# BurntSushi/rust-snappy

Hardware: AMD Instinct MI355X
Metric: GiB/s uncompressed (compress + decompress) on zflat/uflat corpus (higher is better)
Workload: dtype u8

## Files before the change

rust-snappy_amd/csrc/snapmi_api.hip:

```cpp
#include <hip/hip_runtime.h>

#include <cstdarg>
#include <cstdio>
#include <cstdlib>
#include <cstring>
#include <new>
#include <string>
#include <vector>

#include "snapmi.h"
#include "snapmi_test.h"
#include "snapmi_ctx.hpp"
#include "snapmi_launch.hpp"
#include "snapmi_device.hpp"
#include "snapmi_kernels.hpp"

using namespace snapmi;

namespace {

void set_err(snapmi_error *e, int kind, uint64_t a = 0, uint64_t b = 0,
             uint64_t c = 0)
{
    if (e) {
// ... 270 lines not shown
        ctx->small_table_kernel = (int)value;
    else if (strcmp(name, "small_table_min_blocks") == 0 && value >= 1)
        ctx->small_table_min_blocks = (uint64_t)value;
    else if (strcmp(name, "small_batch_kernel") == 0 && value >= 0 &&
             value <= 2)
        ctx->small_batch_kernel = (int)value;
    else if (strcmp(name, "lane_speculate") == 0 && value >= 0 && value <= 1)
        ctx->lane_speculate = (int)value;
    else if (strcmp(name, "lane_tail_probes") == 0 && value >= 0 &&
             value <= 4)
        ctx->lane_tail_probes = (uint32_t)value;
    else if (strcmp(name, "lane_tail_idle_pct") == 0 && value >= 0 &&
             value <= 100)
        ctx->lane_tail_idle_pct = (uint32_t)value;
    else if (strcmp(name, "span_kernel") == 0 && value >= kSpanMin &&
             value <= 1)
        ctx->span_kernel = (int)value;
    else if (strcmp(name, "match_kernel") == 0 && value >= 0 && value <= 2)
        ctx->match_kernel = (int)value;
    else if (strcmp(name, "match_spans_ratio_pct") == 0 && value >= 1 &&
             value <= 200)
        ctx->match_spans_ratio_pct = (uint32_t)value;
    else if (strcmp(name, "release_scratch") == 0 && value >= 0 && value <= 1)
        ctx->release_scratch = (int)value;
    else if (strcmp(name, "batch_long_streams") == 0 && value >= 0 &&
             value <= 1)
        ctx->batch_long_streams = (int)value;
    else if (strcmp(name, "both_wave_cus") == 0 && value >= 0 &&
             value <= 4096)
        ctx->both_wave_cus = (uint32_t)value;
    else if (strcmp(name, "tiny_stream_kernel") == 0 && value >= 0 &&
             value <= 1)
        ctx->tiny_stream_kernel = (int)value;
    else if (strcmp(name, "small_stream_kernel") == 0 && value >= 0 &&
             value <= 2)
        ctx->small_stream_kernel = (int)value;
    else if (strcmp(name, "frame_parallel_walk_min") == 0 && value >= 0)
        ctx->frame_parallel_walk_min = (uint64_t)value;
    else if (strcmp(name, "host_copy_kernel") == 0 && value >= 0 && value <= 3)
        ctx->host_copy_kernel = (int)value;
    else if (strcmp(name, "host_encode_slice") == 0 && value >= (1 << 16))
        ctx->host_encode_slice = (uint64_t)value;
    else if (strcmp(name, "host_decode_slice_chunks") == 0 && value >= 1)
        ctx->host_decode_slice_chunks = (uint64_t)value;
    else if (strcmp(name, "host_batch_slice") == 0 && value >= (1 << 16))
        ctx->host_batch_slice = (uint64_t)value;
    else if (strcmp(name, "range_scratch_bytes") == 0 && value >= (128 << 10))
        ctx->range_scratch_bytes = (uint64_t)value;
    else if (strcmp(name, "write_scratch_bytes") == 0 &&
             value >= (int64_t)(kSlotBytes + kMaxBlock))
        ctx->write_scratch_bytes = (uint64_t)value;
    else if (strcmp(name, "decode_kernel") == 0 &&
             (value == 0 || (value == 2 && kDec2) || value == 3))
        ctx->decode_kernel = ctx->lds_store_order_ok ? (int)value : 0;
    else
        return fail_ctx(ctx, SNAPMI_E_ARGUMENT, "unknown option %s", name);
    return SNAPMI_OK;
}

#ifdef SNAPMI_TESTING
int snapmi_ctx_set_test_option(snapmi_ctx *ctx, const char *name,
                               int64_t value)
{
    if (!ctx || !name)
        return SNAPMI_E_ARGUMENT;
    if (strcmp(name, "lane_waves_per_cu") == 0 && value >= 1 && value <= 32)
        ctx->lane_waves_per_cu = (uint32_t)value;
    else if (strcmp(name, "decode_many_min") == 0 && value >= 0)
        ctx->decode_many_min = (uint64_t)value;
    else if (strcmp(name, "lane_speculate_max_blocks") == 0 && value >= 0)
        ctx->lane_speculate_max_blocks = (uint64_t)value;
    else if (strcmp(name, "lane_max_waves") == 0 && value >= 0 &&
             value <= 0x7FFFFFFF)
        ctx->lane_max_waves = (uint32_t)value;
    else if (strcmp(name, "frame_crc_side_stream") == 0 && value >= 0 &&
             value <= 1)
        ctx->frame_crc_side_stream = value != 0;
    else if (strcmp(name, "lane_tables_uncached") == 0 && value >= 0 &&
             value <= 1)
        ctx->lane_tables_uncached = (int)value;
    else if (strcmp(name, "lane_overlap_encode") == 0 && value >= 0 &&
             value <= 2)
        ctx->lane_overlap_encode = (int)value;
    else if (strcmp(name, "frame_walk_segment") == 0 && value >= (128 << 10))
        ctx->frame_walk_segment = (uint64_t)value;
    else if (strcmp(name, "lane_table_stride_kib") == 0 &&
             (value == 0 || (value >= 256 && value <= 4096 && value % 4 == 0)))
        ctx->lane_table_stride_kib = (uint32_t)value;
    else if (strcmp(name, "lane_table_probe") == 0 && value >= 0 &&
             value <= 1)
        ctx->lane_table_probe = value != 0;
    else if (strcmp(name, "lane_tables_renew") == 0 && value == 1) {
        if (ctx->lane_tables.p) {
            HIP_TRY(ctx, hipStreamSynchronize(ctx->stream));
            snapmi::free_lane_tables(ctx);
        }
    } else if (strcmp(name, "lane_epoch_preset") == 0 && value >= -1 &&
             value <= 0xFFFF)
        ctx->lane_epoch_preset = value;
    else if (strcmp(name, "index_build_route") == 0 && value >= 0 &&
             value <= 2)
        ctx->index_build_route = (uint32_t)value;
    else if (strcmp(name, "index_build_group_streams") == 0 && value >= 1 &&
             value <= 4096)
        ctx->index_build_group_streams = (uint32_t)value;
    else if (strcmp(name, "stream_seg_log2") == 0 &&
             (value == 0 || value == 10 || value == 12))
        ctx->stream_seg_log2 = (uint32_t)value;
    else if (strcmp(name, "stream_scan_segs") == 0 &&
             (value == 0 || value == 8 || value == 16 || value == 32 ||
              value == 64))
        ctx->stream_scan_segs = (uint32_t)value;
    else if (strcmp(name, "lds_order_ok") == 0 && value >= 0 && value <= 1)
        ctx->lds_order_ok = ctx->lds_order_hw && value != 0;
    else if (strcmp(name, "host_batch_direct_min") == 0 && value >= 0)
        ctx->host_batch_direct_min = (uint64_t)value;
    else if (strcmp(name, "host_batch_pack_to_host") == 0 && value >= 0 &&
             value <= 1)
        ctx->host_batch_pack_to_host = (int)value;
    else if (strcmp(name, "host_batch_listed") == 0 && value >= 0 &&
             value <= 1)
        ctx->host_batch_listed = (int)value;
    else
        return fail_ctx(ctx, SNAPMI_E_ARGUMENT, "unknown test option %s",
                        name);
    return SNAPMI_OK;
}
#endif

void *snapmi_host_alloc(size_t bytes)
{
    void *p = nullptr;
    if (hipHostMalloc(&p, bytes ? bytes : 1, hipHostMallocDefault) != hipSuccess) {
        (void)hipGetLastError();
        return nullptr;
    }
    return p;
}

void snapmi_host_free(void *p)
{
    if (p)
        (void)hipHostFree(p);
}

const char *snapmi_table_probe_log(const snapmi_ctx *ctx)
{
    return ctx ? ctx->probe_log.c_str() : "";
}

size_t snapmi_error_string(const snapmi_error *e, char *buf, size_t cap)
{
    char tmp[256];
    const unsigned long long a = e ? e->a : 0, b = e ? e->b : 0,
                             c = e ? e->c : 0;
    int n = 0;
    switch (e ? e->kind : -1) {
    case SNAPMI_TOO_BIG:
        n = snprintf(tmp, sizeof tmp,
                     "snappy: input buffer (size = %llu) is larger than "
                     "allowed (size = %llu)", a, b);
        break;
    case SNAPMI_BUFFER_TOO_SMALL:
        n = snprintf(tmp, sizeof tmp,
                     "snappy: output buffer (size = %llu) is smaller than "
                     "required (size = %llu)", a, b);
// ... 481 lines not shown
```

rust-snappy_amd/csrc/snapmi_compress.hip:

```cpp
#include <type_traits>

#include "snapmi_device.hpp"
#include "snapmi_kernels.hpp"
#include "snapmi_scan.hpp"
#include "snapmi_span.hpp"

namespace snapmi {

namespace {

__device__ __forceinline__ uint32_t hash32(uint32_t x, uint32_t shift)
{
    return (x * 0x1E35A7BDu) >> shift;
}

struct DeltaTable {
    uint32_t d[448];
};
constexpr DeltaTable make_delta()
{
    DeltaTable t{};
    uint32_t skip = 32, p = 0;
    for (int i = 0; i < 448; i++) {
        t.d[i] = p < 0x100000u ? p : 0x100000u;
// ... 161 lines not shown
        o += lt;
        gcptr in = src + P;
        const uint32_t Lp = (L + 15u) & ~15u;
        if (L && L <= 64 && P + Lp <= n) {
            u32x4 v0 = {0, 0, 0, 0}, v1 = v0, v2 = v0, v3 = v0;
            v0 = ld128g(in);
            if (L > 16)
                v1 = ld128g(in + 16);
            if (L > 32)
                v2 = ld128g(in + 32);
            if (L > 48)
                v3 = ld128g(in + 48);
            typedef __attribute__((address_space(1))) u32x4 g_u32x4;
            typedef g_u32x4 __attribute__((aligned(1))) g_u32x4u;
            if (L >= 16)
                *(g_u32x4u *)o = v0;
            if (L >= 32)
                *(g_u32x4u *)(o + 16) = v1;
            if (L >= 48)
                *(g_u32x4u *)(o + 32) = v2;
            if (L >= 64)
                *(g_u32x4u *)(o + 48) = v3;
            const uint32_t pk = L >> 4;
            const u32x4 pv = pk == 0 ? v0 : (pk == 1 ? v1 : (pk == 2 ? v2 : v3));
            gptr po = o + (L & ~15u);
            const uint32_t r = L & 15u;
            if (r >= 4)
                st32u(po, pv.x);
            if (r >= 8)
                st32u(po + 4, pv.y);
            if (r >= 12)
                st32u(po + 8, pv.z);
            const uint32_t tl = r & 3u, tb = r & ~3u;
            const uint32_t ti = r >> 2;
            const uint32_t tw =
                ti == 0 ? pv.x : (ti == 1 ? pv.y : (ti == 2 ? pv.z : pv.w));
            if (tl >= 1)
                po[tb] = (uint8_t)tw;
            if (tl >= 2)
                po[tb + 1] = (uint8_t)(tw >> 8);
            if (tl >= 3)
                po[tb + 2] = (uint8_t)(tw >> 16);
        } else if (L && L <= 64) {
            uint32_t i = 0;
            for (; i + 4 <= L; i += 4)
                st32u(o + i, ld32u(in + i));
            for (; i < L; i++)
                o[i] = in[i];
        }
        gptr oc = o + L;
        const uint8_t olo = (uint8_t)O, ohi = (uint8_t)(O >> 8);
        for (uint32_t i = 0; i < n64; i++) {
            oc[0] = (uint8_t)((63u << 2) | 2u);
            oc[1] = olo;
            oc[2] = ohi;
            oc += 3;
        }
        if (mid) {
            oc[0] = (uint8_t)((59u << 2) | 2u);
            oc[1] = olo;
            oc[2] = ohi;
            oc += 3;
        }
        if (fin == 2) {
            oc[0] = (uint8_t)(((O >> 8) << 5) | ((fin_len - 4) << 2) | 1u);
            oc[1] = olo;
        } else if (fin == 3) {
            oc[0] = (uint8_t)(((fin_len - 1) << 2) | 2u);
            oc[1] = olo;
            oc[2] = ohi;
        }
        uint64_t longs = __ballot(L > 64);
        while (longs) {
            const uint32_t j = (uint32_t)__builtin_ctzll(longs);
            longs &= longs - 1;
            const uint32_t Lj = rdlane(L, j);
            const uint32_t Pj = rdlane(P, j);
            const uint64_t oj = ((uint64_t)rdlane((uint32_t)((uintptr_t)o >> 32), j) << 32) |
                                rdlane((uint32_t)(uintptr_t)o, j);
            wave_copy<true>((gptr)(uintptr_t)oj, src + Pj, Lj, lane);
        }
    }
};

template <class P>
__device__ __forceinline__ uint32_t extend_match(P src, uint32_t n,
                                                 uint32_t c, uint32_t p,
                                                 uint32_t lane)
{
    uint32_t len = 0;
    const uint32_t room = n - p;
    for (uint32_t pos = 0;; pos += 4 * kWave) {
        const uint32_t off = pos + 4 * lane;
        uint32_t eq = 0;
        if (off < room) {
            const uint32_t pa = c + off, pb = p + off;
            const uint32_t ca = pa < n - 4 ? pa : n - 4;
            const uint32_t cb = pb < n - 4 ? pb : n - 4;
            const uint32_t va = ld32u(src + ca) >> (8 * (pa - ca));
            const uint32_t vb = ld32u(src + cb) >> (8 * (pb - cb));
            const uint32_t x = va ^ vb;
            eq = x ? ((uint32_t)__builtin_ctz(x) >> 3) : 4u;
            const uint32_t lim = room - off;
            eq = eq < lim ? eq : lim;
        }
        const uint64_t stop = __ballot(eq < 4);
        if (stop == 0) {
            len += 4 * kWave;
            continue;
        }
        const uint32_t f = (uint32_t)__builtin_ctzll(stop);
        return len + 4 * f + rdlane(eq, f);
    }
}


}

template <bool kLds>
__device__ __forceinline__ void compress_one_block(
    const CompressArgs &a, const uint32_t b, const uint32_t lane,
    const lptr16 table, const uint32_t tbase, const uint32_t c2,
    const uint32_t c3, const uint32_t cB, const uint32_t cBn,
    __attribute__((address_space(3))) uint8_t *lblock = nullptr)
{

    uint32_t lo = 0, hi = a.n_streams;
    if (b < a.n_streams && a.blk_first[b] == b && a.blk_first[b + 1] > b) {
        lo = b;
        hi = b + 1;
    }
    while (hi - lo > 1) {
        const uint32_t mid = (lo + hi) >> 1;
        if (a.blk_first[mid] <= b)
            lo = mid;
        else
            hi = mid;
    }
    const uint32_t st = lo;
    const uint32_t k = b - a.blk_first[st];
    const uint64_t total = a.in_lens[st];
    const uint64_t boff = (uint64_t)k * kMaxBlock;
    gcptr src = (gcptr)a.in_ptrs[st] + boff;
    const uint64_t avail = total - boff;
    const uint32_t n = avail < kMaxBlock ? (uint32_t)avail : kMaxBlock;

    gptr dst;
    if (k == 0) {
        dst = (gptr)a.out_ptrs[st];
        if (lane == 0) {
            uint64_t v = total;
            uint32_t i = 0;
            while (v >= 0x80) {
                dst[i++] = (uint8_t)v | 0x80;
                v >>= 7;
            }
            dst[i] = (uint8_t)v;
        }
        dst += varint_len(total);
    } else {
        const uint32_t slot = a.slot_first[st] + k - 1;
        if (slot >= a.host_slots)
            return;
        dst = (gptr)a.scratch + (uint64_t)slot * kSlotBytes;
    }
    TokenSink out;
// ... 2025 lines not shown
    a.lane_epochs[g] = epoch;
    PROF_TAIL(
    if (a.prof && lane == 0)
        atomicMax(&a.prof[kProfTail + 1], (unsigned long long)wall_clock64());
    )
#ifdef SNAPMI_TESTING
    if (kTail && lane == 0 && multi_rounds)
        atomicAdd(&a.tok_ctl[kTokCtlMultiRounds], multi_rounds);
#endif
}
}

#define SNAPMI_LANE_KERNEL(name, spec, tail)                                  \
    __global__ __launch_bounds__(64) void name(CompressArgs a)                \
    {                                                                         \
        __shared__ __attribute__((aligned(16))) uint32_t ring[kLaneRingWords]; \
        __shared__ __attribute__((aligned(16)))                               \
        unsigned long long tokbuf[kLaneTokWords];                             \
        match_blocks<spec, tail>(                                             \
            a, threadIdx.x, blockIdx.x * 64 + threadIdx.x,                    \
            (__attribute__((address_space(3))) uint32_t *)ring,               \
            (__attribute__((address_space(3))) unsigned long long *)tokbuf);  \
    }
SNAPMI_LANE_KERNEL(k_match_blocks, false, true)
SNAPMI_LANE_KERNEL(k_match_blocks_plain, false, false)
SNAPMI_LANE_KERNEL(k_match_blocks_spec, true, false)
#undef SNAPMI_LANE_KERNEL

namespace {
template <bool kTail>
__device__ __forceinline__ void match_both(
    const CompressArgs &a,
    __attribute__((address_space(3))) uint32_t *const ring,
    __attribute__((address_space(3))) unsigned long long *const tokbuf,
    const lptr16 tables)
{
    const uint32_t lane = threadIdx.x & 63;
    const uint32_t wave = uni(threadIdx.x >> 6);
    if (wave < kBothLaneWaves) {
        match_blocks<false, kTail>(
            a, lane, (blockIdx.x * kBothLaneWaves + wave) * 64 + lane,
            ring + wave * kLaneRingWords, tokbuf + wave * kLaneTokWords);
        return;
    }
    const lptr16 table = tables + (wave - kBothLaneWaves) * kMaxTable;
    const uint32_t tbase = (uint32_t)(uintptr_t)table;
    uint32_t nblocks = a.blk_first[a.n_streams];
    if (nblocks > a.host_blocks)
        nblocks = a.host_blocks;
    if (nblocks > a.blk_hi)
        nblocks = a.blk_hi;
    for (;;) {
        const uint32_t b =
            uni(next_back_ticket(a.ticket, lane, a.blk_lo, nblocks));
        if (b == 0xFFFFFFFFu)
            break;
        compress_one_block_span<false, true>(a, b, lane, table, tbase);
    }
    PROF_TAIL(
    if (a.prof && lane == 0)
        atomicMax(&a.prof[kProfTail + 1], (unsigned long long)wall_clock64());
    )
}
}
#define SNAPMI_BOTH_KERNEL(name, tail)                                        \
    __global__ __launch_bounds__(kBothWaves * 64) void name(CompressArgs a)   \
    {                                                                         \
        __shared__ __attribute__((aligned(16)))                               \
        uint32_t ring[kBothLaneWaves][kLaneRingWords];                        \
        __shared__ __attribute__((aligned(16)))                               \
        unsigned long long tokbuf[kBothLaneWaves][kLaneTokWords];             \
        __shared__ __attribute__((aligned(16)))                               \
        uint16_t tables[kBothWaves - kBothLaneWaves][kMaxTable];              \
        match_both<tail>(                                                     \
            a, (__attribute__((address_space(3))) uint32_t *)&ring[0][0],     \
            (__attribute__((address_space(3))) unsigned long long *)          \
                &tokbuf[0][0],                                                \
            (lptr16)&tables[0][0]);                                           \
    }
SNAPMI_BOTH_KERNEL(k_match_both, true)
SNAPMI_BOTH_KERNEL(k_match_both_plain, false)
#undef SNAPMI_BOTH_KERNEL

__global__ __launch_bounds__(64) void k_encode_tokens(CompressArgs a)
{
    const uint32_t lane = threadIdx.x;
    const uint32_t b = a.blk_lo + blockIdx.x;
    uint32_t nblocks = a.blk_first[a.n_streams];
    if (nblocks > a.host_blocks)
        nblocks = a.host_blocks;
    if (nblocks > a.blk_hi)
        nblocks = a.blk_hi;
    if (b >= nblocks)
        return;
    if (a.ntok[b] >= kTokSpilled)
        return;
    uint32_t lo = 0, hi = a.n_streams;
    if (b < a.n_streams && a.blk_first[b] == b && a.blk_first[b + 1] > b) {
        lo = b;
        hi = b + 1;
    }
    while (hi - lo > 1) {
        const uint32_t mid = (lo + hi) >> 1;
        if (a.blk_first[mid] <= b)
            lo = mid;
        else
            hi = mid;
    }
    const uint32_t st = lo;
    const uint32_t k = b - a.blk_first[st];
    const uint64_t total = a.in_lens[st];
    const uint64_t boff = (uint64_t)k * kMaxBlock;
    gcptr src = (gcptr)a.in_ptrs[st] + boff;
    const uint32_t n =
        total - boff < kMaxBlock ? (uint32_t)(total - boff) : kMaxBlock;
    gptr dst;
    if (k == 0) {
        dst = (gptr)a.out_ptrs[st];
        if (lane == 0) {
            uint64_t v = total;
            uint32_t i = 0;
            while (v >= 0x80) {
                dst[i++] = (uint8_t)v | 0x80;
                v >>= 7;
            }
            dst[i] = (uint8_t)v;
        }
        dst += varint_len(total);
    } else if (a.direct) {
        const uint32_t first = a.blk_first[st];
        const uint64_t nb = (total + kMaxBlock - 1) / kMaxBlock;
        if (first + nb > a.host_blocks)
            return;
        dst = (gptr)a.out_ptrs[st] + varint_len(total) +
              (a.blk_off[b] - a.blk_off[first]);
    } else {
        const uint32_t slot = a.slot_first[st] + k - 1;
        if (slot >= a.host_slots)
            return;
        dst = (gptr)a.scratch + (uint64_t)slot * kSlotBytes;
    }
    TokenSink out;
    out.init(src, n, dst, lane);
    typedef __attribute__((address_space(1))) uint32_t g_tok;
    typedef __attribute__((address_space(1))) unsigned long long g_u64;
    const uint32_t ptab =
        lane < kPageTabStride
            ? a.tok_pages[(uint64_t)(b - a.tok_base) * kPageTabStride + lane]
            : 0;
    const g_tok *const pool = (const g_tok *)a.tok_pool;
    const uint32_t count = a.ntok[b];
    uint32_t pos_base = 0, exc_base = 0;
    uint32_t tnext =
        lane < count ? pool[(uint64_t)rdlane(ptab, 0) * kTokPage + lane] : 0;
    for (uint32_t t0 = 0; t0 < count; t0 += kWave) {
        const uint32_t m = count - t0 < kWave ? count - t0 : kWave;
        uint32_t L = 0, C = 0, O = 0;
        const uint32_t t = tnext;
        if (t0 + kWave < count) {
            const uint32_t pg = rdlane(ptab, (t0 + kWave) / kTokPage);
            if (t0 + kWave + lane < count)
                tnext = pool[(uint64_t)pg * kTokPage +
                             (t0 + kWave) % kTokPage + lane];
        }
        const uint32_t field = (t >> 10) & 63u;
        if (lane < m) {
            L = t & 1023u;
            C = field == kTokLiteral ? 0u : field + 4u;
            O = t >> 16;
        }
        const bool ex = lane < m && field == kTokException;
        const uint64_t E = __builtin_amdgcn_ballot_w64(ex);
        if (E) {
            const uint32_t ei =
                exc_base + __builtin_amdgcn_mbcnt_hi(
                               (uint32_t)(E >> 32),
                               __builtin_amdgcn_mbcnt_lo((uint32_t)E, 0));
            const uint32_t eslot = ei / kExcPage < kExcPagesPerBlock
                                       ? ei / kExcPage
                                       : kExcPagesPerBlock - 1;
            const uint32_t epg = (uint32_t)__builtin_amdgcn_ds_bpermute(
                (int)((kTokPagesPerBlock + eslot) << 2), (int)ptab);
            if (ex) {
                const unsigned long long f =
                    ((const g_u64 *)(pool + (uint64_t)epg * kTokPage))
                        [ei % kExcPage];
                L = (uint32_t)f & 0x1FFFFu;
                C = (uint32_t)(f >> 17) & 0xFFFFu;
                O = (uint32_t)(f >> 33) & 0xFFFFu;
            }
            exc_base += (uint32_t)__builtin_popcountll(E);
        }
        const uint32_t span = L + C;
        const uint32_t incl = wave_inclusive_scan(span);
        const uint32_t P = pos_base + incl - span;
        pos_base += rdlane(incl, kWave - 1);
        out.a = (L & 0xFFFFu) | (O << 16);
        out.b = C | (P << 16);
        out.t = m;
        out.flush();
    }
    if (lane == 0 && !a.direct)
        a.blk_size[b] = out.d;
}

namespace {
__device__ __forceinline__ uint32_t plan_blocks(const CompressArgs &a,
                                                uint32_t i, bool report)
{
    const uint64_t len = a.in_lens[i];
    const uint64_t need = max_compress_len_u64(len);
    if (report)
        a.out_lens[i] = 0;
    if (need == 0) {
        if (report)
            set_error(a.errs, i, SNAPMI_TOO_BIG, len, kMaxInput, 0);
        return 0;
    }
    if (a.out_caps && a.out_caps[i] < need) {
        if (report)
            set_error(a.errs, i, SNAPMI_BUFFER_TOO_SMALL, a.out_caps[i], need,
                      0);
        return 0;
    }
    if (len == 0) {
        if (report) {
            ((gptr)a.out_ptrs[i])[0] = 0;
            a.out_lens[i] = 1;
            set_error(a.errs, i, SNAPMI_OK, 0, 0, 0);
        }
        return 0;
    }
    if (report)
        set_error(a.errs, i, SNAPMI_OK, 0, 0, 0);
    if (len < a.small_limit)
        return 0;
    return (uint32_t)((len + kMaxBlock - 1) / kMaxBlock);
}
__device__ __forceinline__ void plan_load(const CompressArgs &a, uint32_t i,
                                          uint32_t (&x)[2])
{
    x[0] = plan_blocks(a, i, true);
    x[1] = x[0] ? x[0] - 1 : 0;
}
__device__ __forceinline__ void plan_store(const CompressArgs &a, uint32_t i,
                                           uint32_t nb, uint32_t fb,
                                           uint32_t fs)
{
    if (nb && ((uint64_t)fb + nb > a.host_blocks ||
               (uint64_t)fs + (nb - 1) > a.host_slots))
        set_error(a.errs, i, SNAPMI_E_ARGUMENT, a.in_lens[i], 0, 0);
    a.blk_first[i] = fb;
    a.slot_first[i] = fs;
}
}

__global__ __launch_bounds__(1024) void k_plan_compress(CompressArgs a)
{
    uint32_t carry[2] = {0, 0};
    wg_scan_strided(
        a.n_streams, carry,
        [&](uint32_t i, uint32_t (&x)[2]) { plan_load(a, i, x); },
        [&](uint32_t i, const uint32_t (&x)[2], const uint32_t (&ex)[2]) {
            plan_store(a, i, x[0], ex[0], ex[1]);
        });
    if (threadIdx.x == 0) {
        a.blk_first[a.n_streams] = carry[0];
        a.slot_first[a.n_streams] = carry[1];
    }
}

namespace {
__device__ __forceinline__ uint32_t scan_nblocks(const CompressArgs &a)
{
    uint32_t nblocks = a.blk_first[a.n_streams];
    if (nblocks > a.host_blocks)
        nblocks = a.host_blocks;
    if (nblocks > a.blk_hi)
        nblocks = a.blk_hi;
    return nblocks;
}
}

__global__ __launch_bounds__(1024) void k_scan_sizes(CompressArgs a)
{
    const uint32_t nblocks = scan_nblocks(a);
// ... 221 lines not shown
```

rust-snappy_amd/csrc/snapmi_ctx.hpp:

```cpp
#pragma once

#include <hip/hip_runtime.h>

#include <cstdarg>
#include <cstdio>
#include <string>
#include <vector>

#include "snapmi.h"

namespace snapmi {

struct DevBuf {
    void *p = nullptr;
    size_t cap = 0;
    bool listed = false;
};

struct PinBuf {
    void *p = nullptr;
    size_t cap = 0;
    bool listed = false;
};

}

struct snapmi_host_pipe;

struct snapmi_ctx {
    int device = 0;
    snapmi_host_pipe *pipe = nullptr;
    volatile uint32_t *h_mail = nullptr;
    std::vector<snapmi::DevBuf *> dev_bufs;
    std::vector<snapmi::PinBuf *> pin_bufs;
    snapmi::PinBuf pin_in, pin_out, pin_desc;
    uint64_t host_encode_slice = 2048ull << 20;
    uint64_t host_decode_slice_chunks = 8192;
    int host_copy_kernel = 1;
    uint64_t host_batch_slice = 16ull << 20;
    uint64_t host_batch_direct_min = 1ull << 20;
    int host_batch_pack_to_host = 1;
    int host_batch_listed = 1;
    uint64_t hb_slices = 0, hb_h2d_bytes = 0, hb_d2h_bytes = 0;
    uint64_t hb_listed_slices = 0;
    hipStream_t stream = nullptr;
    bool owns_stream = false;
    std::string last_error;
    snapmi::DevBuf blk_first, slot_first, blk_size, blk_off, slots, plan_part;
    snapmi::DevBuf tokens, tok_pages, tok_stage, ntok, lane_tables,
        lane_epochs;
    std::vector<hipMemGenericAllocationHandle_t> lane_chunks;
    size_t lane_chunk_bytes = 0, lane_va_bytes = 0;
    uint32_t lane_chunk_count = 0, lane_per_chunk = 0;
    uint32_t n_lanes = 0;
    uint64_t lane_stride = 0;
    bool lane_table_spread = true;
    bool lane_tables_top = false;
    int compress_mode = 1;
    int span_schedule = 1;
    snapmi::DevBuf sched;
    int lane_coresident = 1;
    uint64_t lane_coresident_min_blocks = 98304;
    const char *last_kernel = "";
    int small_table_kernel = 1;
    uint64_t small_table_min_blocks = 256;
    int small_batch_kernel = 1;
    int span_kernel = 1;
    uint32_t both_wave_cus = 0;
    int release_scratch = 0;
    int match_kernel = 2;
    uint32_t match_spans_ratio_pct = 90;
    volatile uint32_t *h_ratio = nullptr;
    uint32_t ratio_seq = 0;
    uint32_t token_pool_pct = 39, token_pool_now = 0;
    uint32_t token_pool_min_pages = 32768;
    volatile uint32_t *h_tokstat = nullptr;
    uint32_t tokstat_seq = 0, tokstat_seen = 0;
    uint32_t tok_pages_asked = 0, tok_blocks_spilled = 0;
    uint32_t tok_pool_pages_last = 0;
    int lane_speculate = 1;
    uint64_t lane_speculate_max_blocks = 24576;
    uint32_t lane_tail_probes = 2;
    uint32_t lane_tail_idle_pct = 40;
    int tiny_stream_kernel = 1;
    int small_stream_kernel = 1;
    uint64_t decode_many_min = 1u << 20;
    int lane_overlap_encode = 0;
    int lane_tables_uncached = 0;
    int decode_kernel = 3;
    hipStream_t stream2 = nullptr;
    hipEvent_t ev_fork = nullptr, ev_join = nullptr;
    hipEvent_t ev_crc[2] = {nullptr, nullptr};
    bool frame_crc_side_stream = true;
    snapmi::DevBuf st_in, st_out, st_desc, st_prof, ticket, order;
    snapmi::DevBuf sd_tables, sd_desc;
    int batch_long_streams = 1;
    snapmi::DevBuf bl_modes, bl_list, bl_descs, bl_order;
    snapmi::PinBuf pin_bl;
    snapmi::PinBuf pin_bl2;
    snapmi::DevBuf ix_modes, ix_desc, ix_gate;
    uint64_t ix_seq = 0;
    bool ix_stats_live = false;
    snapmi::DevBuf rg_desc, rg_meta, rg_part, rg_room, rg_stat;
    uint64_t range_scratch_bytes = 1ull << 30;
    uint64_t rg_pieces = 0;
    bool rg_stats_live = false;
    snapmi::DevBuf ib_meta, ib_stat;
    snapmi::PinBuf pin_ib, pin_ibg[2];
    hipEvent_t ev_ib = nullptr, ev_ibg[2] = {nullptr, nullptr};
    bool ev_ib_live = false, ev_ibg_live[2] = {false, false};
    uint64_t ib_groups = 0;
    bool ib_stats_live = false;
    snapmi::DevBuf wr_meta, wr_state, wr_z, wr_slot, wr_room, wr_desc, wr_stat;
    snapmi::PinBuf pin_wr;
    hipEvent_t ev_wr = nullptr;
    bool ev_wr_live = false;
    uint64_t write_scratch_bytes = 1ull << 30;
    uint64_t wr_blocks = 0, wr_decoded = 0;
    bool wr_stats_live = false;
    snapmi::DevBuf ap_meta, ap_state, ap_stat;
    snapmi::PinBuf pin_ap;
    hipEvent_t ev_ap = nullptr;
    bool ev_ap_live = false;
    uint64_t ap_blocks = 0, ap_decoded = 0;
    bool ap_stats_live = false;
    uint32_t index_build_route = 0;
    uint32_t index_build_group_streams = 4096;
    uint32_t stream_seg_log2 = 0;
    uint32_t stream_scan_segs = 0;
    snapmi::DevBuf fr_tables, fr_desc, fr_scan, fr_slots, fr_chunk_off;
    snapmi::DevBuf fr_crc;
    snapmi::DevBuf fb_streams, fb_chunks;
    bool fr_tables_ready = false;
    uint64_t frame_parallel_walk_min = 4ull << 20;
    uint64_t frame_walk_segment = 32ull << 20;
    int num_cus = 0;
    hipEvent_t ev[6] = {nullptr, nullptr, nullptr, nullptr, nullptr, nullptr};
    uint32_t lane_min_blocks = 20480;
    uint32_t lane_segment_blocks = 262144;
    uint32_t lane_waves_per_cu = 6;
    uint32_t lane_max_waves = 0;
    uint32_t lane_table_tries = 2;
    uint32_t lane_table_budget_pct = 33;
    bool lane_table_probe = false;
    uint32_t lane_table_stride_kib = 0;
    std::string probe_log;
    int64_t lane_epoch_preset = -1;
    bool lds_order_ok = false;
    bool lds_order_hw = false;
    bool lds_store_order_ok = true;
    bool timing_valid = false;
    bool timing_is_compress = false;
    bool dominant_split = false;
    uint64_t codec_launches = 0;
    uint32_t seam_seq = 0;
    uint32_t prof_tail_lanes = 0;
};

namespace snapmi {

inline int fail_ctx(snapmi_ctx *ctx, int kind, const char *fmt, ...)
{
    char buf[512];
    va_list ap;
    va_start(ap, fmt);
    vsnprintf(buf, sizeof buf, fmt, ap);
    va_end(ap);
    if (ctx)
        ctx->last_error = buf;
    return kind;
// ... 33 lines not shown
```

rust-snappy_amd/csrc/snapmi_kernels.hpp:

```cpp
#pragma once

#include <hip/hip_runtime.h>
#include <stdint.h>

#include "snapmi.h"
#include "snapmi_tiny.hpp"
#include "snapmi_profile.hpp"
#include "snapmi_streamplan.hpp"
#include "snapmi_blockindex.hpp"

namespace snapmi {

struct CompressArgs {
    const void *const *in_ptrs;
    const uint64_t *in_lens;
    void *const *out_ptrs;
    const uint64_t *out_caps;
    uint64_t *out_lens;
    snapmi_error *errs;
    uint32_t *blk_first;
    uint32_t *slot_first;
    uint32_t *blk_size;
    uint64_t *blk_off;
    uint8_t *scratch;
// ... 39 lines not shown
static_assert(kTokPagesPerBlock + kExcPagesPerBlock <= kPageTabStride, "");
constexpr uint32_t kPagesPerSmallBlock = (8192 / 4 + 64 + kTokPage - 1) / kTokPage + 1;
constexpr uint32_t kTokCtlList = 16;
constexpr uint32_t kProfTail = 16, kProfTailLanes = 32;
constexpr uint32_t kTicketIdle = 2;
constexpr uint32_t kTokCtlMultiRounds = 4;
constexpr uint32_t kTokStageWords = kMaxTokens + 2 * (kMaxTokens / 16) + 28;
constexpr uint32_t kTokSpilled = 0xFFFFFFFEu;
constexpr uint32_t kTokLiteral = 61, kTokException = 62;
#if defined(__HIPCC__)
__device__ __forceinline__ bool tok_fits(uint32_t lit, uint32_t copy)
{
    return lit <= 1023u && copy <= 64u;
}
__device__ __forceinline__ uint32_t tok_pack(uint32_t lit, uint32_t copy,
                                             uint32_t offset)
{
    const uint32_t field = copy ? copy - 4u : kTokLiteral;
    return tok_fits(lit, copy) ? (offset << 16) | (field << 10) | lit
                               : kTokException << 10;
}
__device__ __forceinline__ unsigned long long tok_pack64(uint32_t lit,
                                                         uint32_t copy,
                                                         uint32_t offset)
{
    return (unsigned long long)lit | ((unsigned long long)copy << 17) |
           ((unsigned long long)offset << 33);
}
#endif

struct DecompressArgs {
    const void *const *in_ptrs;
    const uint64_t *in_lens;
    void *const *out_ptrs;
    const uint64_t *out_caps;
    uint64_t *out_lens;
    snapmi_error *errs;
    const uint8_t *modes;
    const unsigned long long *gate;
    unsigned long long gate_value;
    uint32_t n_streams;
    uint32_t *order;
    uint32_t *bucket_pos;
    unsigned long long *prof;
};

__global__ void k_probe_lds_order(uint32_t *bad);
__global__ void k_zero16(unsigned long long *p, unsigned long long n);
__global__ void k_seam_compress_tiny(const uint8_t *in, uint32_t n,
                                     uint8_t *out,
                                     unsigned long long *out_len,
                                     uint32_t *done, uint32_t seq);
__global__ void k_seam_decompress_tiny(DecompressArgs a, uint32_t *done,
                                       uint32_t seq);
__global__ void k_probe_tables(unsigned long long *tables,
                               unsigned long long stride, uint32_t steps,
                               uint32_t chunks, uint32_t per_chunk);
__global__ void k_plan_compress(CompressArgs a);
__global__ void k_plan_compress_a(CompressArgs a);
__global__ void k_plan_compress_b(CompressArgs a, uint32_t nparts);
__global__ void k_plan_compress_c(CompressArgs a);
__global__ void k_scan_sizes_a(CompressArgs a, uint32_t nparts);
__global__ void k_scan_sizes_b(CompressArgs a, uint32_t nparts);
__global__ void k_scan_sizes_c(CompressArgs a);
__global__ void k_compress_blocks(CompressArgs a);
__global__ void k_compress_block_lds(CompressArgs a);
__global__ void k_compress_spans(CompressArgs a);
__global__ void k_match_spans(CompressArgs a);
__global__ void k_redo_spilled(CompressArgs a, uint32_t *h_stat, uint32_t seq);
__global__ void k_match_spans_8k(CompressArgs a);
__global__ void k_post_ratio(uint32_t *host_mapped, const uint64_t *blk_off,
                             uint32_t blocks, const uint64_t *in_lens,
                             uint32_t n_streams, uint32_t seq);
__global__ void k_compress_span_lds(CompressArgs a);
__global__ void k_compress_tiny(CompressArgs a);
__global__ void k_compress_small512(CompressArgs a);
__global__ void k_compress_small1k(CompressArgs a);
__global__ void k_compress_small2k(CompressArgs a);
__global__ void k_match_blocks(CompressArgs a);
__global__ void k_match_blocks_spec(CompressArgs a);
__global__ void k_match_both(CompressArgs a);
__global__ void k_match_blocks_plain(CompressArgs a);
__global__ void k_match_both_plain(CompressArgs a);
__global__ void k_encode_tokens(CompressArgs a);
__global__ void k_scan_sizes(CompressArgs a);
__global__ void k_compact(CompressArgs a);
__global__ void k_stream_lens(CompressArgs a);

struct StreamArgs {
    const uint8_t *in;
    unsigned long long in_len;
    uint8_t *out;
    unsigned long long out_cap;
    unsigned long long *out_len;
    snapmi_error *err;
    unsigned long long *meta;
    unsigned long long *s1, *s2, *s3;
    unsigned long long *e1, *e2, *e3;
    unsigned long long *cuts;
    uint32_t nseg, nsuper, nsuper3, kmax;
    uint32_t seg_log2;
    uint32_t scan_segs;
    const void **c_in;
    unsigned long long *c_inlen;
    void **c_out;
    unsigned long long *c_cap;
    unsigned long long *c_outlen;
    snapmi_error *c_err;
    uint8_t *c_mode;
    uint8_t *fb_mode;
};
struct BatchStreams {
    const StreamArgs *descs;
    const uint32_t *pre;
    uint32_t n;
};
__host__ __device__ inline bool long_stream_rule(unsigned long long len,
                                                 unsigned long long dl,
                                                 unsigned long long min_len)
{
    const bool sane = dl / 22 <= len && 2 * dl >= 3ull * kStreamChunk;
    return sane && len >= min_len &&
           (2 * dl >= 3 * len || len >= (256ull << 10));
}
struct LongItem {
    uint32_t idx, pad;
    unsigned long long in_len, dlen;
    const void *in;
    void *out;
    unsigned long long out_cap;
};
#define SNAPMI_STREAM_KERNEL_DECL(name)                                       \
    __global__ void k_bstream_##name(BatchStreams b);
SNAPMI_STREAM_KERNEL_DECL(head)
SNAPMI_STREAM_KERNEL_DECL(scan)
SNAPMI_STREAM_KERNEL_DECL(super)
SNAPMI_STREAM_KERNEL_DECL(super3)
SNAPMI_STREAM_KERNEL_DECL(chain)
SNAPMI_STREAM_KERNEL_DECL(spread3)
SNAPMI_STREAM_KERNEL_DECL(spread2)
SNAPMI_STREAM_KERNEL_DECL(cuts)
SNAPMI_STREAM_KERNEL_DECL(pieces)
SNAPMI_STREAM_KERNEL_DECL(finish)
__global__ void k_long_plan(const void *const *in_ptrs, const uint64_t *in_lens,
                            void *const *out_ptrs, const uint64_t *out_caps,
                            uint32_t n, uint64_t min_len, uint8_t *modes,
                            LongItem *list, uint32_t cap, uint32_t *count);

struct IndexArgs {
    const void *const *in_ptrs;
    const uint64_t *in_lens;
    void *const *out_ptrs;
    const uint64_t *out_caps;
    uint64_t *out_lens;
    snapmi_error *errs;
    const uint64_t *first;
    const uint64_t *index;
    uint64_t entries;
    uint32_t n;
    uint8_t *modes;
    const void **c_in;
    uint64_t *c_inlen;
    void **c_out;
    uint64_t *c_cap;
    uint64_t *c_outlen;
    snapmi_error *c_err;
    uint8_t *c_mode;
// ... 188 lines not shown
```

rust-snappy_amd/csrc/snapmi_launch.hip:

```cpp
#include <hip/hip_runtime.h>

#include <cstdio>
#include <cstring>
#include <vector>

#include "snapmi.h"
#include "snapmi_test.h"
#include "snapmi_ctx.hpp"
#include "snapmi_launch.hpp"
#include "snapmi_pool.hpp"
#include "snapmi_route.hpp"
#include "snapmi_device.hpp"
#include "snapmi_kernels.hpp"

using namespace snapmi;

namespace snapmi {
static_assert(kRouteCompressWaves == kCompressWaves &&
                  kRouteSmallTableWaves == kSmallTableWaves &&
                  kRouteBothWaves == kBothWaves &&
                  kRouteBothLaneWaves == kBothLaneWaves &&
                  kRouteTinyCompress == kTinyCompress &&
                  kRouteSmallCompress == kSmallCompress,
              "snapmi_route.hpp and snapmi_kernels.hpp disagree");
// ... 366 lines not shown
                    100;
                a.lane_tail_depth = ctx->lane_tail_probes;
                a.lane_tail_idle = ctx->lane_tail_idle_pct == 0 ? 0
                                   : idle                       ? (uint32_t)idle
                                                                : 1;
            }
        }
    }
    a.prof = nullptr;
    PROF(
    if ((rc = reserve(ctx, ctx->st_prof, 16 * sizeof(uint64_t))))
        return rc;
    HIP_TRY(ctx, hipMemsetAsync(ctx->st_prof.p, 0, 16 * sizeof(uint64_t),
                                ctx->stream));
    a.prof = (unsigned long long *)ctx->st_prof.p;
    )
    PROF_TAIL(
    {
        const size_t bytes =
            (size_t)(kProfTailLanes + route.lanes) * sizeof(uint64_t);
        if ((rc = reserve(ctx, ctx->st_prof, bytes)))
            return rc;
        HIP_TRY(ctx, hipMemsetAsync(ctx->st_prof.p, 0, bytes, ctx->stream));
        a.prof = (unsigned long long *)ctx->st_prof.p;
        ctx->prof_tail_lanes = route.lanes;
    }
    )

    hipStream_t s = ctx->stream;
    ctx->timing_valid = false;
    HIP_TRY(ctx, hipEventRecord(ctx->ev[0], s));
    launch_scan(
        n,
        [&] {
            hipLaunchKernelGGL(k_plan_compress, dim3(1), dim3(1024), 0, s, a);
        },
        [&](uint32_t parts) {
            hipLaunchKernelGGL(k_plan_compress_a, dim3(parts), dim3(1024), 0,
                               s, a);
            hipLaunchKernelGGL(k_plan_compress_b, dim3(1), dim3(1024), 0, s, a,
                               parts);
            hipLaunchKernelGGL(k_plan_compress_c, dim3(parts), dim3(1024), 0,
                               s, a);
        });
    HIP_TRY(ctx, hipEventRecord(ctx->ev[1], s));
    {
        const dim3 grid((uint32_t)((n + 63) / 64));
        if (a.small_limit && (small_classes & 1))
            hipLaunchKernelGGL(k_compress_tiny, grid, dim3(64), 0, s, a);
        if (a.small_limit > kTinyCompress) {
            if (small_classes & 2)
                hipLaunchKernelGGL(k_compress_small512, grid, dim3(64), 0, s,
                                   a);
            if (small_classes & 4)
                hipLaunchKernelGGL(k_compress_small1k, grid, dim3(64), 0, s,
                                   a);
            if (small_classes & 8)
                hipLaunchKernelGGL(k_compress_small2k, grid, dim3(64), 0, s,
                                   a);
        }
    }
    if (route.window != WindowKernel::none) {
        HIP_TRY(ctx, hipMemsetAsync(ctx->ticket.p, 0, 64, s));
        hipStream_t ws = s;
        if (route.window_beside) {
            HIP_TRY(ctx, hipEventRecord(ctx->ev_fork, s));
            HIP_TRY(ctx, hipStreamWaitEvent(ctx->stream2, ctx->ev_fork, 0));
            ws = ctx->stream2;
        }
        if (route.sched) {
            const size_t head = (size_t)(16 + n) * 4;
            const size_t lists = (size_t)2 * (slots + 1) * 4;
            if ((rc = reserve(ctx, ctx->sched, head + lists)))
                return rc;
            HIP_TRY(ctx, hipMemsetAsync(ctx->sched.p, 0, head, ws));
            HIP_TRY(ctx, hipMemsetAsync((uint8_t *)ctx->sched.p + head, 0xFF,
                                        lists, ws));
            a.sched = (uint32_t *)ctx->sched.p;
        }
        launch_window(route, a, ws);
        a.sched = nullptr;
    }
    if (route.tokens) {
        HIP_TRY(ctx, hipEventRecord(ctx->ev[4], s));
        for (uint64_t lo = 0; lo < blocks; lo += route.seg_blocks) {
            const uint64_t hi = lo + route.seg_blocks < blocks
                                    ? lo + route.seg_blocks
                                    : blocks;
            const Segment g = segment(o, route, lo, hi);
            a.tok_base = (uint32_t)lo;
            a.blk_lo = (uint32_t)lo;
            a.blk_hi = (uint32_t)g.mid;
            HIP_TRY(ctx, hipMemsetAsync(ctx->tok_pages.p, 0,
                                        kTokCtlList * 4, s));
            if (route.window == WindowKernel::none)
                HIP_TRY(ctx, hipMemsetAsync(ctx->ticket.p, 0, 64, s));
            a.cls_lo = route.small_grid ? 8192 : 0;
            launch_match(o, route, g, a, s);
            if (route.small_grid) {
                HIP_TRY(ctx, hipMemsetAsync(ctx->ticket.p, 0, 64, s));
                a.cls_lo = 0;
                a.cls_hi = 8192;
                hipLaunchKernelGGL(k_match_spans_8k, dim3(route.small_grid),
                                   dim3(kSmallTableWaves * 64), 0, s, a);
            }
            a.cls_lo = 0;
            a.cls_hi = kMaxBlock;
            if (g.mid < hi) {
                HIP_TRY(ctx, hipEventRecord(ctx->ev_fork, s));
                HIP_TRY(ctx,
                        hipStreamWaitEvent(ctx->stream2, ctx->ev_fork, 0));
                hipLaunchKernelGGL(k_encode_tokens,
                                   dim3((uint32_t)(g.mid - lo)), dim3(64), 0,
                                   ctx->stream2, a);
                HIP_TRY(ctx, hipEventRecord(ctx->ev_join, ctx->stream2));
                a.blk_lo = (uint32_t)g.mid;
                a.blk_hi = (uint32_t)hi;
                HIP_TRY(ctx, hipMemsetAsync(ctx->ticket.p, 0, 64, s));
                launch_match(o, route, g, a, s);
            }
            if (hi == blocks)
                HIP_TRY(ctx, hipEventRecord(ctx->ev[5], s));
            if (route.window_beside) {
                HIP_TRY(ctx, hipEventRecord(ctx->ev_join, ctx->stream2));
                HIP_TRY(ctx, hipStreamWaitEvent(s, ctx->ev_join, 0));
            }
            if (route.direct)
                launch_scan_sizes(a, s);
            hipLaunchKernelGGL(k_encode_tokens,
                               dim3((uint32_t)(hi - a.blk_lo)), dim3(64), 0, s,
                               a);
            if (g.mid < hi)
                HIP_TRY(ctx, hipStreamWaitEvent(s, ctx->ev_join, 0));
            if (!ctx->h_tokstat) {
                HIP_TRY(ctx, hipHostMalloc((void **)&ctx->h_tokstat, 64,
                                           hipHostMallocDefault));
                memset((void *)ctx->h_tokstat, 0, 64);
            }
            CompressArgs r = a;
            r.blk_lo = (uint32_t)lo;
            r.blk_hi = (uint32_t)hi;
            r.cls_lo = 0;
            r.cls_hi = kMaxBlock;
            hipLaunchKernelGGL(k_redo_spilled, dim3(g.redo_grid),
                               dim3(kCompressWaves * 64), 0, s, r,
                               (uint32_t *)ctx->h_tokstat, ++ctx->tokstat_seq);
        }
        a.blk_lo = 0;
        a.tok_base = 0;
        a.blk_hi = (uint32_t)blocks;
    }
    HIP_TRY(ctx, hipEventRecord(ctx->ev[2], s));
    if (route.direct) {
        hipLaunchKernelGGL(k_stream_lens, dim3((uint32_t)((n + 255) / 256)),
                           dim3(256), 0, s, a);
        if (route.post_ratio) {
            if (!ctx->h_ratio) {
                HIP_TRY(ctx, hipHostMalloc((void **)&ctx->h_ratio, 64,
                                           hipHostMallocDefault));
                memset((void *)ctx->h_ratio, 0, 64);
            }
            hipLaunchKernelGGL(k_post_ratio, dim3(1), dim3(1024), 0, s,
                               (uint32_t *)ctx->h_ratio, a.blk_off,
                               (uint32_t)blocks, a.in_lens, a.n_streams,
                               ++ctx->ratio_seq);
        }
    } else if (blocks) {
        launch_scan_sizes(a, s);
        hipLaunchKernelGGL(k_compact, dim3((uint32_t)blocks), dim3(256), 0,
                           s, a);
    }
    if (d_index_first) {
        uint64_t *part = (uint64_t *)ctx->plan_part.p;
        launch_scan(
            n,
            [&] {
                hipLaunchKernelGGL(k_index_first, dim3(1), dim3(1024), 0, s,
                                   d_in_lens, (uint32_t)n, d_index_first);
            },
            [&](uint32_t parts) {
                hipLaunchKernelGGL(k_index_first_a, dim3(parts), dim3(1024), 0,
                                   s, d_in_lens, (uint32_t)n, d_index_first,
                                   part);
                hipLaunchKernelGGL(k_index_first_b, dim3(1), dim3(1024), 0, s,
                                   (uint32_t)n, d_index_first, part, parts);
                hipLaunchKernelGGL(k_index_first_c, dim3(parts), dim3(1024), 0,
                                   s, (uint32_t)n, d_index_first, part);
            });
        if (index_entries)
            hipLaunchKernelGGL(k_block_index,
                               dim3((uint32_t)((index_entries + 255) / 256)),
                               dim3(256), 0, s, a, d_index_first, d_index,
                               index_entries);
    }
    HIP_TRY(ctx, hipEventRecord(ctx->ev[3], s));
    HIP_TRY(ctx, hipGetLastError());
    ctx->timing_valid = true;
    ctx->timing_is_compress = true;
    ctx->last_kernel = route.last_kernel;
    ctx->dominant_split = route.tokens;
    ctx->codec_launches = blocks ? 1 : 0;
    return SNAPMI_OK;
}

int launch_decompress(snapmi_ctx *ctx, const void *const *d_in_ptrs,
                      const uint64_t *d_in_lens, void *const *d_out_ptrs,
                      const uint64_t *d_out_caps, uint64_t *d_out_lens,
                      snapmi_error *d_errs, const uint8_t *d_modes, size_t n,
                      const unsigned long long *d_gate,
                      unsigned long long gate_value, hipStream_t side,
                      DevBuf *side_order, bool wide_only)
{
    HIP_TRY(ctx, hipSetDevice(ctx->device));
    DevBuf &order = side_order ? *side_order : ctx->order;
// ... 90 lines not shown
```

Measured before the change: 125.5.

## Stage encoded token output in LDS and write aligned 16-byte lines

```diff
diff --git a/rust-snappy_amd/csrc/snapmi_api.hip b/rust-snappy_amd/csrc/snapmi_api.hip
--- a/rust-snappy_amd/csrc/snapmi_api.hip
+++ b/rust-snappy_amd/csrc/snapmi_api.hip
@@ -376,6 +376,8 @@
     else if (strcmp(name, "lane_overlap_encode") == 0 && value >= 0 &&
              value <= 2)
         ctx->lane_overlap_encode = (int)value;
+    else if (strcmp(name, "encode_lines") == 0 && value >= 0 && value <= 1)
+        ctx->encode_lines = (int)value;
     else if (strcmp(name, "frame_walk_segment") == 0 && value >= (128 << 10))
         ctx->frame_walk_segment = (uint64_t)value;
     else if (strcmp(name, "lane_table_stride_kib") == 0 &&
diff --git a/rust-snappy_amd/csrc/snapmi_compress.hip b/rust-snappy_amd/csrc/snapmi_compress.hip
--- a/rust-snappy_amd/csrc/snapmi_compress.hip
+++ b/rust-snappy_amd/csrc/snapmi_compress.hip
@@ -267,6 +267,146 @@
         }
     }
 };
+
+constexpr uint32_t kStageBytes = 4096;
+typedef __attribute__((address_space(3))) uint8_t l_u8;
+struct LineSink {
+    TokenSink s;
+    l_u8 *stage;
+    uint32_t fill, own;
+
+    __device__ __forceinline__ void init(gcptr src, uint32_t len, gptr o,
+                                         uint32_t l, l_u8 *st)
+    {
+        s.init(src, len, o, l);
+        stage = st;
+        fill = own = uni((uint32_t)(uintptr_t)o & 15u);
+    }
+
+    __device__ __forceinline__ void drain()
+    {
+        if (fill > own) {
+            gptr base = s.dst + s.d - fill;
+            if (s.lane >= own && s.lane < fill)
+                base[s.lane] = stage[s.lane];
+        }
+    }
+
+    __device__ __forceinline__ void flush()
+    {
+        const uint32_t lane = s.lane;
+        const bool act = lane < s.t;
+        const uint32_t C = act ? (s.b & 0xFFFFu) : 0;
+        uint32_t L = act ? (s.a & 0xFFFFu) : 0;
+        if (act && L == 0 && C == 0)
+            L = kMaxBlock;
+        const uint32_t O = s.a >> 16;
+        const uint32_t P = s.b >> 16;
+        const uint32_t lt = L == 0 ? 0 : (L <= 60 ? 1 : (L <= 256 ? 2 : 3));
+        const uint32_t n64 = C >= 68 ? (C - 4) >> 6 : 0;
+        const uint32_t rem = C - (n64 << 6);
+        const uint32_t mid = rem > 64 ? 1 : 0;
+        const uint32_t fin_len = rem - 60 * mid;
+        const bool c1 = fin_len <= 11 && O <= 2047;
+        const uint32_t fin = C == 0 ? 0 : (c1 ? 2 : 3);
+        const uint32_t size = lt + L + 3 * (n64 + mid) + fin;
+        const uint32_t incl = wave_inclusive_scan(size);
+        const uint32_t total = rdlane(incl, kWave - 1);
+        const uint32_t Lp = (L + 15u) & ~15u;
+        const bool odd = L > 64 || (L && P + Lp > s.n);
+        if (fill + total > kStageBytes || __ballot(odd) != 0) {
+            drain();
+            s.flush();
+            fill = own = uni((uint32_t)(uintptr_t)(s.dst + s.d) & 15u);
+            return;
+        }
+        s.t = 0;
+        typedef __attribute__((address_space(3))) u32x4 l_u32x4;
+        l_u8 *const o = stage + fill + (incl - size);
+        if (__ballot(L != 0) != 0) {
+            gcptr in = s.src + P;
+            u32x4 v0 = {0, 0, 0, 0}, v1 = v0, v2 = v0, v3 = v0;
+            if (L)
+                v0 = ld128g(in);
+            if (L > 16)
+                v1 = ld128g(in + 16);
+            if (L > 32)
+                v2 = ld128g(in + 32);
+            if (L > 48)
+                v3 = ld128g(in + 48);
+            l_u8 *const ol = o + lt;
+            if (L > 48)
+                __builtin_memcpy(ol + 48, &v3, 16);
+            __builtin_amdgcn_wave_barrier();
+            if (L > 32)
+                __builtin_memcpy(ol + 32, &v2, 16);
+            __builtin_amdgcn_wave_barrier();
+            if (L > 16)
+                __builtin_memcpy(ol + 16, &v1, 16);
+            __builtin_amdgcn_wave_barrier();
+            if (L)
+                __builtin_memcpy(ol, &v0, 16);
+            __builtin_amdgcn_wave_barrier();
+        }
+        if (lt) {
+            const uint32_t n1 = L - 1;
+            if (lt == 1) {
+                o[0] = (uint8_t)(n1 << 2);
+            } else {
+                o[0] = lt == 2 ? (60u << 2) : (61u << 2);
+                o[1] = (uint8_t)n1;
+                if (lt == 3)
+                    o[2] = (uint8_t)(n1 >> 8);
+            }
+        }
+        l_u8 *oc = o + lt + L;
+        const uint8_t olo = (uint8_t)O, ohi = (uint8_t)(O >> 8);
+        for (uint32_t i = 0; i < n64; i++) {
+            oc[0] = (uint8_t)((63u << 2) | 2u);
+            oc[1] = olo;
+            oc[2] = ohi;
+            oc += 3;
+        }
+        if (mid) {
+            oc[0] = (uint8_t)((59u << 2) | 2u);
+            oc[1] = olo;
+            oc[2] = ohi;
+            oc += 3;
+        }
+        if (fin == 2) {
+            oc[0] = (uint8_t)(((O >> 8) << 5) | ((fin_len - 4) << 2) | 1u);
+            oc[1] = olo;
+        } else if (fin == 3) {
+            oc[0] = (uint8_t)(((fin_len - 1) << 2) | 2u);
+            oc[1] = olo;
+            oc[2] = ohi;
+        }
+        __builtin_amdgcn_wave_barrier();
+        const uint32_t end = fill + total;
+        const uint32_t nl = end >> 4;
+        if (nl) {
+            gptr base = s.dst + s.d - fill;
+            if (own && lane >= own && lane < 16)
+                base[lane] = stage[lane];
+            typedef __attribute__((address_space(1))) u32x4 g_u32x4;
+            for (uint32_t i = lane + (own ? 1u : 0u); i < nl; i += kWave)
+                *(g_u32x4 *)(base + 16 * i) = *(const l_u32x4 *)(stage + 16 * i);
+            const u32x4 c = *(const l_u32x4 *)(stage + 16 * nl);
+            __builtin_amdgcn_wave_barrier();
+            if (lane == 0)
+                *(l_u32x4 *)stage = c;
+            __builtin_amdgcn_wave_barrier();
+            fill = end & 15u;
+            own = 0;
+        } else {
+            fill = end;
+        }
+        s.d += total;
+    }
+};
+
+__device__ __forceinline__ TokenSink &sink_tokens(TokenSink &s) { return s; }
+__device__ __forceinline__ TokenSink &sink_tokens(LineSink &s) { return s.s; }
 
 template <class P>
 __device__ __forceinline__ uint32_t extend_match(P src, uint32_t n,
@@ -2458,7 +2598,10 @@
 SNAPMI_BOTH_KERNEL(k_match_both_plain, false)
 #undef SNAPMI_BOTH_KERNEL
 
-__global__ __launch_bounds__(64) void k_encode_tokens(CompressArgs a)
+namespace {
+template <bool kLines>
+__device__ __forceinline__ void encode_tokens(const CompressArgs &a,
+                                              l_u8 *const stage)
 {
     const uint32_t lane = threadIdx.x;
     const uint32_t b = a.blk_lo + blockIdx.x;
@@ -2516,8 +2659,11 @@
             return;
         dst = (gptr)a.scratch + (uint64_t)slot * kSlotBytes;
     }
-    TokenSink out;
-    out.init(src, n, dst, lane);
+    typename std::conditional<kLines, LineSink, TokenSink>::type out;
+    if constexpr (kLines)
+        out.init(src, n, dst, lane, stage);
+    else
+        out.init(src, n, dst, lane);
     typedef __attribute__((address_space(1))) uint32_t g_tok;
     typedef __attribute__((address_space(1))) unsigned long long g_u64;
     const uint32_t ptab =
@@ -2571,13 +2717,26 @@
         const uint32_t incl = wave_inclusive_scan(span);
         const uint32_t P = pos_base + incl - span;
         pos_base += rdlane(incl, kWave - 1);
-        out.a = (L & 0xFFFFu) | (O << 16);
-        out.b = C | (P << 16);
-        out.t = m;
+        TokenSink &tok = sink_tokens(out);
+        tok.a = (L & 0xFFFFu) | (O << 16);
+        tok.b = C | (P << 16);
+        tok.t = m;
         out.flush();
     }
+    if constexpr (kLines)
+        out.drain();
     if (lane == 0 && !a.direct)
-        a.blk_size[b] = out.d;
+        a.blk_size[b] = sink_tokens(out).d;
+}
+}
+__global__ __launch_bounds__(64) void k_encode_tokens(CompressArgs a,
+                                                      uint32_t lines)
+{
+    extern __shared__ __attribute__((aligned(16))) uint8_t encode_stage[];
+    if (lines)
+        encode_tokens<true>(a, (l_u8 *)encode_stage);
+    else
+        encode_tokens<false>(a, nullptr);
 }
 
 namespace {
diff --git a/rust-snappy_amd/csrc/snapmi_ctx.hpp b/rust-snappy_amd/csrc/snapmi_ctx.hpp
--- a/rust-snappy_amd/csrc/snapmi_ctx.hpp
+++ b/rust-snappy_amd/csrc/snapmi_ctx.hpp
@@ -86,6 +86,7 @@
     int small_stream_kernel = 1;
     uint64_t decode_many_min = 1u << 20;
     int lane_overlap_encode = 0;
+    int encode_lines = 1;
     int lane_tables_uncached = 0;
     int decode_kernel = 3;
     hipStream_t stream2 = nullptr;
diff --git a/rust-snappy_amd/csrc/snapmi_kernels.hpp b/rust-snappy_amd/csrc/snapmi_kernels.hpp
--- a/rust-snappy_amd/csrc/snapmi_kernels.hpp
+++ b/rust-snappy_amd/csrc/snapmi_kernels.hpp
@@ -145,7 +145,8 @@
 __global__ void k_match_both(CompressArgs a);
 __global__ void k_match_blocks_plain(CompressArgs a);
 __global__ void k_match_both_plain(CompressArgs a);
-__global__ void k_encode_tokens(CompressArgs a);
+constexpr uint32_t kEncodeStageLds = 4096 + 16;
+__global__ void k_encode_tokens(CompressArgs a, uint32_t lines);
 __global__ void k_scan_sizes(CompressArgs a);
 __global__ void k_compact(CompressArgs a);
 __global__ void k_stream_lens(CompressArgs a);
diff --git a/rust-snappy_amd/csrc/snapmi_launch.hip b/rust-snappy_amd/csrc/snapmi_launch.hip
--- a/rust-snappy_amd/csrc/snapmi_launch.hip
+++ b/rust-snappy_amd/csrc/snapmi_launch.hip
@@ -472,6 +472,7 @@
         a.sched = nullptr;
     }
     if (route.tokens) {
+        const uint32_t lines = ctx->encode_lines && ctx->lds_order_ok ? 1 : 0;
         HIP_TRY(ctx, hipEventRecord(ctx->ev[4], s));
         for (uint64_t lo = 0; lo < blocks; lo += route.seg_blocks) {
             const uint64_t hi = lo + route.seg_blocks < blocks
@@ -501,8 +502,9 @@
                 HIP_TRY(ctx,
                         hipStreamWaitEvent(ctx->stream2, ctx->ev_fork, 0));
                 hipLaunchKernelGGL(k_encode_tokens,
-                                   dim3((uint32_t)(g.mid - lo)), dim3(64), 0,
-                                   ctx->stream2, a);
+                                   dim3((uint32_t)(g.mid - lo)), dim3(64),
+                                   lines ? kEncodeStageLds : 0, ctx->stream2,
+                                   a, lines);
                 HIP_TRY(ctx, hipEventRecord(ctx->ev_join, ctx->stream2));
                 a.blk_lo = (uint32_t)g.mid;
                 a.blk_hi = (uint32_t)hi;
@@ -518,8 +520,8 @@
             if (route.direct)
                 launch_scan_sizes(a, s);
             hipLaunchKernelGGL(k_encode_tokens,
-                               dim3((uint32_t)(hi - a.blk_lo)), dim3(64), 0, s,
-                               a);
+                               dim3((uint32_t)(hi - a.blk_lo)), dim3(64),
+                               lines ? kEncodeStageLds : 0, s, a, lines);
             if (g.mid < hi)
                 HIP_TRY(ctx, hipStreamWaitEvent(s, ctx->ev_join, 0));
             if (!ctx->h_tokstat) {
```

After: 123.2. 0.982x the previous value.
